# otiliastr/coper

Measured on AMD Instinct MI355X. Metric: scored triples/sec (1-vs-all), higher is better.
Workload: dtype fp16x3 (fp32 values split into two fp16 terms, 3 fp16 MFMAs per product, fp32 accumulate; comparisons closer than the split's error decided by the fp32 chain)

## Files before the change

### coper_amd/csrc/kernels_dense_fused_bf16.hip

```cpp
#include "bf16x3_chain.h"
#include "coper_internal.h"
#ifdef COPER_DBG_GROUP_CLK
#include <hip/hip_runtime.h>
__device__ unsigned long long g_group_clk[8];
extern "C" __attribute__((visibility("default"))) int coper_dbg_group_clock(unsigned long long* out) {
  return hipMemcpyFromSymbol(out, HIP_SYMBOL(g_group_clk), sizeof(unsigned long long) * 8) == hipSuccess ? 0 : 1;
}
#define GROUP_CLK(i) do { __syncthreads(); if (threadIdx.x == 0) g_group_clk[i] = wall_clock64(); } while (0)
#endif
#include "group_body.h"
#include "conv_fold.h"

namespace coper {

typedef float f32x4 __attribute__((ext_vector_type(4)));
typedef unsigned u32x4 __attribute__((ext_vector_type(4)));

#define MFMA16_BF16(a, b, c) S16_MFMA16(a, b, c)
#define MFMA16_X3(ahi, alo, bhi, blo, c) \
  { (c) = MFMA16_BF16(alo, bhi, c); (c) = MFMA16_BF16(ahi, blo, c); (c) = MFMA16_BF16(ahi, bhi, c); }


#ifndef COPER_FUSED_PMAX
#define COPER_FUSED_PMAX 3
#endif
#ifndef COPER_FUSED_PBUDGET
#define COPER_FUSED_PBUDGET 220
#endif


#define FW_DECL u32x4 W[P][NW][2]
#define FW_HI(s_, j_) W[s_][j_][0]
#define FW_LO(s_, j_) W[s_][j_][1]
#define FW_LO_RAW(s_, j_) W[s_][j_][1]
#define FW_PRE(s_)
#define FW_WREG3 (3 * NW * 8)

struct FusedConvArgs {
  const float* e1_rows;
  const int32_t* sorted_row;
  const int32_t* sorted_rid;
  const float* ent;
  const float* rel_emb;
  const float* conv_w;
  const float* conv_b;
  const float* scale;
  const float* shift;
  int per_rel_conv, d, r, in_w, in_hw, Wo, img_stride, x_exp;
  int img_exp;
  int64_t* chk;
  int w_div, w_rem;
  int32_t* bad;
};

#ifdef COPER_DBG_FUSED_CLOCK
__device__ unsigned long long g_fused_ph[8 * 2048];
extern "C" __attribute__((visibility("default"))) int coper_dbg_fused_phases(unsigned long long* out, int n) {
  return hipMemcpyFromSymbol(out, HIP_SYMBOL(g_fused_ph), sizeof(unsigned long long) * 8 * (n < 2048 ? n : 2048)) == hipSuccess ? 0 : 1;
}
#define FUSED_PH(i_)                                                                                            \
  do {                                                                                                          \
    const int w_ = blockIdx.x + gridDim.x * (blockIdx.y + gridDim.y * blockIdx.z);                              \
    if ((threadIdx.x & 63) == 0 && w_ < 2048) g_fused_ph[8 * w_ + (i_)] = __builtin_amdgcn_s_memrealtime();     \
  } while (0)
#else
#define FUSED_PH(i_) do { } while (0)
#endif
struct FusedFinConst {
  const int32_t* perm; const float* fc_b; const float* scale; const float* shift; const int32_t* w_exp; float* x3m;
  int per_rel_bias, x_exp, d, pad;
};
struct FusedFin {
  float* h_out; const FusedFinConst* c;
};
constexpr int FUSED_STAGE_WGS = 16;


__device__ __forceinline__ void fused_load_images(unsigned* __restrict__ img, const FusedConvArgs& A, int start, int n,
                                                  int t0, int t1) {
  const int wave = __builtin_amdgcn_readfirstlane(threadIdx.x >> 6), lane = threadIdx.x & 63;
  const int q0 = wave * 16;
  if (q0 < n) {
    int qi = q0 + (lane & 15);
    if (qi > n - 1) qi = n - 1;
    int my_row = A.sorted_row[start + qi], my_rid = A.sorted_rid[start + qi];
#ifdef COPER_DBG_NO_GROUP_CHK
    const bool chk = false;
#else
    const bool chk = A.chk != nullptr && (blockIdx.y | blockIdx.z) == 0;
#endif
    int64_t live_rel = 0, live_e1 = 0;
    const int chk_row = my_row, chk_rid = my_rid;
    if (chk) group_chk_issue(A.chk, start + qi, live_rel, live_e1);
#ifdef COPER_DBG_FUSED_NO_IMG
    my_row = -1;
#endif
    const float* base = A.e1_rows ? A.e1_rows : A.ent;
    const int len = t1 - t0, PD = (A.img_stride - 1) >> 1, eI = A.img_exp;
    auto fetch2 = [&](const int row, const int rid, const int t) -> float2 {
      if (t >= t1) return make_float2(0.f, 0.f);
      if (t < A.d) return row >= 0 ? *(const float2*)(base + (int64_t)row * A.d + t) : make_float2(0.f, 0.f);
      return *(const float2*)(A.rel_emb + (int64_t)rid * A.r + (t - A.d));
    };
    auto put2 = [&](const int q, const int pp, const float2 x) {
      unsigned short h0, l0, h1, l1;
      split1_s16(x3_scale(x.x, eI), h0, l0);
      split1_s16(x3_scale(x.y, eI), h1, l1);
      img[q * A.img_stride + pp] = (unsigned)h0 | ((unsigned)h1 << 16);
      img[q * A.img_stride + PD + pp] = (unsigned)l0 | ((unsigned)l1 << 16);
    };
    float2 v[16][2];
#pragma unroll
    for (int u = 0; u < 16; ++u) {
      const int row = __builtin_amdgcn_readlane(my_row, u), rid = __builtin_amdgcn_readlane(my_rid, u);
#pragma unroll
      for (int h = 0; h < 2; ++h) v[u][h] = fetch2(row, rid, t0 + 2 * (lane + 64 * h));
    }
#pragma unroll
    for (int u = 0; u < 16; ++u)
      if (q0 + u < n) {
#pragma unroll
        for (int h = 0; h < 2; ++h)
          if (2 * (lane + 64 * h) < len) put2(q0 + u, lane + 64 * h, v[u][h]);
        if (lane == 0) img[(q0 + u) * A.img_stride + 2 * PD] = 0u;
      }
    if (len > 256) {
      for (int u = 0; u < 16 && q0 + u < n; ++u) {
        const int row = __builtin_amdgcn_readlane(my_row, u), rid = __builtin_amdgcn_readlane(my_rid, u);
        for (int pp = 128 + lane; 2 * pp < len; pp += 64) put2(q0 + u, pp, fetch2(row, rid, t0 + 2 * pp));
      }
    }
    if (chk) group_chk_verdict(A.chk, live_rel, live_e1, chk_row, chk_rid);
  }
  asm volatile("s_waitcnt lgkmcnt(0)" ::: "memory");
  __builtin_amdgcn_s_barrier();
}

typedef unsigned fused_img_t;
template <int NFB, int NB, bool WNT>
__device__ __forceinline__ void fused_matrix_role(const uint4* __restrict__ xring, fused_img_t* __restrict__ img,
                                                  const uint4* __restrict__ Whi, const uint4* __restrict__ Wlo,
                                                  const FusedConvArgs& A, int64_t relw, int64_t relw_w, int start, int n, int fb0,
                                                  int nfb, int64_t ks32n, int64_t kb, int64_t ke, int t0, int t1,
                                                  float* __restrict__ zdst, int d_pad16, int wave, const FusedFin& Fn, int64_t ks32s) {
  constexpr int NFULL = NFB / 4;
  constexpr int REM = NFB % 4 ? 1 : 0;
  static_assert(NFB % 4 <= 1, "at most one left-over feature block");
  constexpr int NRQ = REM ? (NB + 3) / 4 : 0;
  constexpr int NW = NFULL + REM;
  constexpr int P = (COPER_FUSED_PMAX >= 3 && (NFULL * NB + NRQ) * 4 + FW_WREG3 + 44 <= COPER_FUSED_PBUDGET) ? 3 : 2;
  constexpr int XSTAGE = 2 * NB * 64;
  const int lane = threadIdx.x & 63;
  const int nk = (int)(ke - kb);
  const uint4* wp[NW][2];
#pragma unroll
  for (int j = 0; j < NW; ++j) {
    int fb = fb0 + (j < NFULL ? wave + 4 * j : 4 * NFULL);
    if (fb > nfb - 1) fb = nfb - 1;
    int64_t o = ((relw_w * nfb + fb) * ks32s + kb) * 64;
    wp[j][0] = Whi + o;
    wp[j][1] = (const uint4*)(Wlo + o);
  }
  FW_DECL;
#define FUSED_W_LOAD(p_) (WNT ? __builtin_nontemporal_load(p_) : *(p_))
#define W_ISSUE(s, kk)                                                                                 \
  {                                                                                                    \
    _Pragma("unroll") for (int j = 0; j < NW; ++j) {                                                   \
      FW_HI(s, j) = FUSED_W_LOAD((const u32x4*)(wp[j][0] + (int64_t)(kk)*64) + lane);                 \
      FW_LO_RAW(s, j) = FUSED_W_LOAD((const u32x4*)((const uint4*)wp[j][1] + (int64_t)(kk)*64) + lane); \
    }                                                                                                  \
  }
#pragma unroll
  for (int t = 0; t < P; ++t)
    if (t < nk) W_ISSUE(t, t);
  if (wave == 0) FUSED_PH(0);
  fused_load_images(img, A, start, n, t0, t1);
  if (wave == 0) FUSED_PH(1);
  f32x4 acc[NFULL][NB], accr[NRQ > 0 ? NRQ : 1];
#pragma unroll
  for (int j = 0; j < NFULL; ++j)
#pragma unroll
    for (int q = 0; q < NB; ++q) acc[j][q] = (f32x4){0.f, 0.f, 0.f, 0.f};
#pragma unroll
  for (int t = 0; t < NRQ; ++t) accr[t] = (f32x4){0.f, 0.f, 0.f, 0.f};
#ifdef COPER_DBG_FUSED_NO_MFMA
#define M_STEP(s2)                                                                                  \
  {                                                                                                 \
    __builtin_amdgcn_s_barrier();                                                                   \
    const uint4* xb = xring + ((s2)&1) * XSTAGE + lane;                                             \
    _Pragma("unroll") for (int j = 0; j < NW; ++j) {                                                \
      acc[0][0][0] += __uint_as_float(FW_HI((s2) % P, j)[0] ^ FW_LO_RAW((s2) % P, j)[1]);           \
      acc[0][0][1] += __uint_as_float(FW_HI((s2) % P, j)[2] ^ FW_LO_RAW((s2) % P, j)[0]);           \
    }                                                                                               \
    acc[0][0][2] += __uint_as_float(xb[0].x);                                                       \
  }
#else
#ifdef COPER_DBG_FUSED_NO_XREAD
#define M_LD(i_) make_uint4((unsigned)lane, (unsigned)(i_), 0x3c003c00u, 0x3c003c00u)
#else
#define M_LD(i_) xb[i_]
#endif
#ifndef COPER_FUSED_XPF
#define COPER_FUSED_XPF 2
#endif
#ifndef COPER_FUSED_XBUDGET
#define COPER_FUSED_XBUDGET 220
#endif
  constexpr int NV = NB + (NRQ > 0 ? 1 : 0);
  constexpr int XPF = (P == 3 && (NFULL * NB + NRQ) * 4 + FW_WREG3 + 44 > COPER_FUSED_XBUDGET) ? 1 : COPER_FUSED_XPF, XR = XPF + 1;
  const int qr = wave < NB ? wave : NB - 1;
#define M_LDV_H(v_) M_LD(((v_) < NB ? (v_) : qr) * 64)
#define M_LDV_L(v_) M_LD((NB + ((v_) < NB ? (v_) : qr)) * 64)
#define M_STEP(s2)                                                                                  \
  {                                                                                                 \
    FW_PRE((s2) % P)                                                                                \
    __builtin_amdgcn_s_barrier();                                                                   \
    const uint4* xb = xring + ((s2)&1) * XSTAGE + lane;                                             \
    uint4 bhq[XR], blq[XR];                                                                         \
    _Pragma("unroll") for (int v = 0; v < XPF && v < NV; ++v) { bhq[v] = M_LDV_H(v); blq[v] = M_LDV_L(v); } \
    __builtin_amdgcn_sched_group_barrier(0x100, 2 * (XPF < NV ? XPF : NV), 0);                      \
    _Pragma("unroll") for (int q = 0; q < NB; ++q) {                                                \
      if (q + XPF < NV) {                                                                           \
        bhq[(q + XPF) % XR] = M_LDV_H(q + XPF); blq[(q + XPF) % XR] = M_LDV_L(q + XPF);             \
        __builtin_amdgcn_sched_group_barrier(0x100, 2, 0);                                          \
      }                                                                                             \
      __builtin_amdgcn_sched_group_barrier(0x008, 3 * NFULL, 0);                                    \
      const uint4 bh = bhq[q % XR], bl = blq[q % XR];                                               \
      _Pragma("unroll") for (int j = 0; j < NFULL; ++j)                                             \
          acc[j][q] = MFMA16_BF16(FW_LO((s2) % P, j), bh, acc[j][q]);                               \
      _Pragma("unroll") for (int j = 0; j < NFULL; ++j)                                             \
          acc[j][q] = MFMA16_BF16(FW_HI((s2) % P, j), bl, acc[j][q]);                               \
      _Pragma("unroll") for (int j = 0; j < NFULL; ++j)                                             \
          acc[j][q] = MFMA16_BF16(FW_HI((s2) % P, j), bh, acc[j][q]);                               \
    }                                                                                               \
    _Pragma("unroll") for (int t = 0; t < NRQ; ++t) {                                               \
      const int q = wave + 4 * t < NB ? wave + 4 * t : NB - 1;  \
      uint4 bh, bl;                                                                                 \
      if (t == 0) { bh = bhq[NB % XR]; bl = blq[NB % XR]; }     \
      else { bh = M_LD(q * 64); bl = M_LD((NB + q) * 64); }                                         \
      accr[t] = MFMA16_BF16(FW_LO((s2) % P, NFULL), bh, accr[t]);                                   \
      accr[t] = MFMA16_BF16(FW_HI((s2) % P, NFULL), bl, accr[t]);                                   \
      accr[t] = MFMA16_BF16(FW_HI((s2) % P, NFULL), bh, accr[t]);                                   \
    }                                                                                               \
  }
#endif
  int k0 = 0;
  for (; k0 + 2 * P <= nk; k0 += 2 * P) {
#pragma unroll
    for (int s2 = 0; s2 < 2 * P; ++s2) {
      M_STEP(s2);
#ifndef COPER_DBG_FUSED_NO_W
      const int kn = k0 + s2 + P;
      W_ISSUE(s2 % P, kn < nk ? kn : 0);
#endif
    }
    if (k0 == 0 && wave == 0) FUSED_PH(2);
  }
#pragma unroll
  for (int s2 = 0; s2 < 2 * P - 1; ++s2) {
    if (k0 + s2 < nk) {
      M_STEP(s2);
#ifndef COPER_DBG_FUSED_NO_W
      if (k0 + s2 + P < nk) W_ISSUE(s2 % P, k0 + s2 + P);
#endif
    }
  }
#undef M_STEP
#undef W_ISSUE
  if (wave == 0) FUSED_PH(3);
#ifdef COPER_DBG_FUSED_NO_STORE
  if (acc[0][0][0] != 1.2345f) return;
#endif
  if (Fn.h_out) {
    const FusedFinConst Fc = *Fn.c;
    const int d = Fc.d;
    const int zexp = -((Fc.w_exp ? Fc.w_exp[Fc.per_rel_bias ? relw : 0] : 0) + Fc.x_exp);
    const float* bsrc = Fc.per_rel_bias ? Fc.fc_b + relw * d : Fc.fc_b;
    float m = 0.f;
    int qrow[NB];
#pragma unroll
    for (int q = 0; q < NB; ++q) {
      const int qi = q * 16 + (lane & 15);
      qrow[q] = qi < n ? Fc.perm[start + qi] : -1;
    }
    auto fin = [&](const f32x4& a, const int fb, const int q, const float4& b4, const float4& s4, const float4& t4) {
      const int k0 = fb * 16 + 4 * (lane >> 4);
      if (fb >= nfb || qrow[q] < 0 || k0 >= d) return;
      float z0 = 0.f, z1 = 0.f, z2 = 0.f, z3 = 0.f;
      z0 += a[0]; z1 += a[1]; z2 += a[2]; z3 += a[3];
      float4 v;
      v.x = fmaxf(fmaf(x3_scale(z0, zexp) + b4.x, s4.x, t4.x), 0.f);
      v.y = fmaxf(fmaf(x3_scale(z1, zexp) + b4.y, s4.y, t4.y), 0.f);
      v.z = fmaxf(fmaf(x3_scale(z2, zexp) + b4.z, s4.z, t4.z), 0.f);
      v.w = fmaxf(fmaf(x3_scale(z3, zexp) + b4.w, s4.w, t4.w), 0.f);
      m = fmaxf(m, fmaxf(fmaxf(v.x, v.y), fmaxf(v.z, v.w)));
      *(float4*)(Fn.h_out + (int64_t)qrow[q] * d + k0) = v;
    };
    auto quad = [&](const float* p, const int fb) -> float4 {
      const int k0 = fb * 16 + 4 * (lane >> 4);
      return (fb < nfb && k0 < d) ? *(const float4*)(p + k0) : make_float4(0.f, 0.f, 0.f, 0.f);
    };
#pragma unroll
    for (int j = 0; j < NFULL; ++j) {
      const int fb = fb0 + wave + 4 * j;
      const float4 b4 = quad(bsrc, fb), s4 = quad(Fc.scale, fb), t4 = quad(Fc.shift, fb);
#pragma unroll
      for (int q = 0; q < NB; ++q) fin(acc[j][q], fb, q, b4, s4, t4);
    }
    if (NRQ > 0) {
      const int fb = fb0 + 4 * NFULL;
      const float4 b4 = quad(bsrc, fb), s4 = quad(Fc.scale, fb), t4 = quad(Fc.shift, fb);
#pragma unroll
      for (int t = 0; t < NRQ; ++t) {
        const int q = wave + 4 * t;
        if (q < NB) {
          const int qi = q * 16 + (lane & 15);
          const int row = qi < n ? Fc.perm[start + qi] : -1;
          const int k0 = fb * 16 + 4 * (lane >> 4);
          if (fb < nfb && row >= 0 && k0 < d) {
            float z0 = 0.f, z1 = 0.f, z2 = 0.f, z3 = 0.f;
            z0 += accr[t][0]; z1 += accr[t][1]; z2 += accr[t][2]; z3 += accr[t][3];
            float4 v;
            v.x = fmaxf(fmaf(x3_scale(z0, zexp) + b4.x, s4.x, t4.x), 0.f);
            v.y = fmaxf(fmaf(x3_scale(z1, zexp) + b4.y, s4.y, t4.y), 0.f);
            v.z = fmaxf(fmaf(x3_scale(z2, zexp) + b4.z, s4.z, t4.z), 0.f);
            v.w = fmaxf(fmaf(x3_scale(z3, zexp) + b4.w, s4.w, t4.w), 0.f);
            m = fmaxf(m, fmaxf(fmaxf(v.x, v.y), fmaxf(v.z, v.w)));
            *(float4*)(Fn.h_out + (int64_t)row * d + k0) = v;
          }
        }
      }
    }
#pragma unroll
    for (int o = 32; o >= 1; o >>= 1) m = fmaxf(m, __shfl_xor(m, o));
    if (lane == 0 && m > 0.f)
      atomicMax((unsigned*)&Fc.x3m[(blockIdx.x + gridDim.x * blockIdx.z) & (X3M_SLOTS - 1)], __float_as_uint(m));
    return;
  }
#pragma unroll
  for (int j = 0; j < NFULL; ++j) {
    const int fb = fb0 + wave + 4 * j;
#pragma unroll
    for (int q = 0; q < NB; ++q) {
      const int qi = q * 16 + (lane & 15);
      if (fb < nfb && qi < n) {
        float* dst = zdst + (int64_t)(start + qi) * d_pad16 + fb * 16 + 4 * (lane >> 4);
        *(float4*)dst = make_float4(acc[j][q][0], acc[j][q][1], acc[j][q][2], acc[j][q][3]);
      }
    }
  }
#pragma unroll
  for (int t = 0; t < NRQ; ++t) {
    const int fb = fb0 + 4 * NFULL, q = wave + 4 * t;
    const int qi = q * 16 + (lane & 15);
    if (fb < nfb && q < NB && qi < n) {
      float* dst = zdst + (int64_t)(start + qi) * d_pad16 + fb * 16 + 4 * (lane >> 4);
      *(float4*)dst = make_float4(accr[t][0], accr[t][1], accr[t][2], accr[t][3]);
    }
  }
}

template <int NB>
__device__ __forceinline__ void fused_conv_role(uint4* __restrict__ xring, unsigned* __restrict__ img,
                                                const FusedConvArgs& A, int64_t relw, int start, int n, int64_t kb,
                                                int64_t ke, int i_lo, int t0, int t1, int cw) {
  constexpr int NFR = (NB + 3) / 4;
  constexpr int XSTAGE = 2 * NB * 64;
  const int lane = threadIdx.x & 63;
  const int nk = (int)(ke - kb);
  const int Wo = A.Wo, in_w = A.in_w, W2 = in_w >> 1;
  const int g = lane >> 4, m = lane & 15;
  const int PD = (A.img_stride - 1) >> 1;
  u32x4 aop[2];
  f32x4 cop[2];
  {
    const float* wsrc = A.per_rel_conv ? A.conv_w + relw * (int64_t)(9 * 32) : A.conv_w;
    const float* bsrc = A.per_rel_conv ? A.conv_b + relw * (int64_t)32 : A.conv_b;
    const int te = A.x_exp - A.img_exp;
#pragma unroll
    for (int u = 0; u < 2; ++u) {
      const int ch = 8 * (m >> 2) + 4 * u + (m & 3);
      const float sc = A.scale[ch];
      unsigned short th[9], tl[9];
#pragma unroll
      for (int k = 0; k < 9; ++k) split1_s16(x3_scale(wsrc[k * 32 + ch] * sc, te), th[k], tl[k]);
      unsigned short sl[8];
#pragma unroll
      for (int k = 0; k < 8; ++k) sl[k] = g == 2 ? tl[k] : th[k];
      if (g == 3) {
        sl[0] = th[8]; sl[1] = th[8]; sl[2] = tl[8];
#pragma unroll
        for (int k = 3; k < 8; ++k) sl[k] = 0;
      }
#pragma unroll
      for (int k = 0; k < 4; ++k) aop[u][k] = (unsigned)sl[2 * k] | ((unsigned)sl[2 * k + 1] << 16);
#pragma unroll
      for (int i = 0; i < 4; ++i) {
        const int c = 8 * g + 4 * u + i;
        cop[u][i] = x3_scale(fmaf(bsrc[c], A.scale[c], A.shift[c]), A.x_exp);
      }
    }
  }
  fused_load_images(img, A, start, n, t0, t1);
  if (cw == 0) FUSED_PH(5);
  int qown[NFR], qoth[NFR];
#pragma unroll
  for (int t = 0; t < NFR; ++t) {
    int qi = (cw + 4 * t) * 16 + m;
    if (qi > n - 1) qi = n - 1;
    qown[t] = qi * A.img_stride + (g == 1 ? PD : 0);
    qoth[t] = qi * A.img_stride + (g == 1 ? 0 : PD);
  }
  int poff = (int)(kb - (int64_t)i_lo * Wo);
  int cj = poff;
  for (int kk = 0; kk <= nk; ++kk) {
    if (kk > 0) {
      asm volatile("s_waitcnt lgkmcnt(0)" ::: "memory");
      __builtin_amdgcn_s_barrier();
    }
#ifdef COPER_DBG_FUSED_NO_CONV
    if (kk < 1) {
#else
    if (kk < nk) {
#endif
      const int pd = poff >> 1;
      const unsigned sh = (unsigned)(poff & 1) << 4;
#pragma unroll
      for (int t = 0; t < NFR; ++t) {
        if (cw + 4 * t < NB) {
          const unsigned* r = img + qown[t] + pd;
          const unsigned d00 = r[0], d01 = r[1], d10 = r[W2], d11 = r[W2 + 1], d20 = r[2 * W2], d21 = r[2 * W2 + 1];
          const unsigned o21 = img[qoth[t] + pd + 2 * W2 + 1];
          const unsigned a01 = __builtin_amdgcn_alignbit(d01, d00, sh), a2 = d01 >> sh;
          const unsigned b01 = __builtin_amdgcn_alignbit(d11, d10, sh), b2 = d11 >> sh;
          const unsigned c01 = __builtin_amdgcn_alignbit(d21, d20, sh), c2 = d21 >> sh;
          u32x4 bop;
          bop[0] = a01;
          bop[1] = __builtin_amdgcn_perm(b01, a2, 0x05040100u);
          bop[2] = __builtin_amdgcn_perm(b2, b01, 0x05040302u);
          bop[3] = c01;
          if (g == 3) {
            bop[0] = __builtin_amdgcn_perm(o21 >> sh, c2, 0x05040100u);
            bop[1] = c2 & 0xffffu;
          }
          const f32x4 y0 = MFMA16_BF16(aop[0], bop, cop[0]);
          const f32x4 y1 = MFMA16_BF16(aop[1], bop, cop[1]);
          float y[8];
#pragma unroll
          for (int i = 0; i < 4; ++i) {
            y[i] = __builtin_amdgcn_fmed3f(y0[i], 0.f, 65504.f);
            y[4 + i] = __builtin_amdgcn_fmed3f(y1[i], 0.f, 65504.f);
          }
          uint4 h4, l4;
          split8_pos_s16(y, h4, l4);
          uint4* dst = xring + (kk & 1) * XSTAGE + (cw + 4 * t) * 64 + lane;
          dst[0] = h4;
          dst[NB * 64] = l4;
        }
      }
      if (++cj == Wo) { cj = 0; poff += in_w - Wo + 1; } else { ++poff; }
    }
  }
}

#ifdef COPER_DBG_FUSED_CLOCK
__device__ unsigned long long g_fused_clk[3 * 2048];
extern "C" __attribute__((visibility("default"))) int coper_dbg_fused_clock(unsigned long long* out, int n) {
  return hipMemcpyFromSymbol(out, HIP_SYMBOL(g_fused_clk), sizeof(unsigned long long) * 3 * (n < 2048 ? n : 2048)) == hipSuccess ? 0 : 1;
}
#endif

template <int NFB, bool WNT>
__global__ __launch_bounds__(512) void k_dense_fused_bf16x3(const uint4* __restrict__ Whi, const uint4* __restrict__ Wlo,
                                                            FusedConvArgs A, const int32_t* __restrict__ tiles,
                                                            const int32_t* __restrict__ n_tiles, int64_t cap_small,
                                                            int nfb, int64_t ks32n, int nslices, int64_t Bcap,
                                                            int d_pad16, float* __restrict__ z_part, FusedFin Fn,
                                                            int n_special, const int32_t* __restrict__ stage_src, int64_t stage_n,
                                                            int64_t* __restrict__ stage_dst, int64_t ks32s, GroupJob J, int n_group,
                                                            const int32_t* __restrict__ post_src, int64_t post_n, int32_t* __restrict__ post_dst) {
  extern __shared__ uint4 fused_lds[];
  if ((int)blockIdx.x < n_special) {
    if (blockIdx.y | blockIdx.z) return;
    const int n_copy = n_special - n_group;
    if ((int)blockIdx.x >= n_copy) {
      GROUP_CLK(0);
      if (J.wait_for > 0) {
        if (threadIdx.x == 0) {
          for (int spin = 0; spin < (1 << 21) && __hip_atomic_load(J.ticket, __ATOMIC_RELAXED, __HIP_MEMORY_SCOPE_AGENT) < J.wait_for; ++spin)
            __builtin_amdgcn_s_sleep(16);
          (void)__hip_atomic_load(J.ticket, __ATOMIC_ACQUIRE, __HIP_MEMORY_SCOPE_AGENT);
          __hip_atomic_store(J.ticket, 0, __ATOMIC_RELAXED, __HIP_MEMORY_SCOPE_AGENT);
        }
        __syncthreads();
      }
      GROUP_CLK(1);
      group_role_body<512>(J, (int*)fused_lds);
      GROUP_CLK(5);
      return;
    }
    const int64_t nb = n_copy, b = (int64_t)blockIdx.x;
    if (post_n > 0) {
      const bool pvec = ((((uintptr_t)post_src) | ((uintptr_t)post_dst)) & 15) == 0;
      const int64_t p4 = pvec ? post_n / 4 : 0;
      for (int64_t i = b * 512 + threadIdx.x; i < p4; i += nb * 512) ((int4*)post_dst)[i] = ((const int4*)post_src)[i];
      for (int64_t i = 4 * p4 + b * 512 + threadIdx.x; i < post_n; i += nb * 512) post_dst[i] = post_src[i];
    }
    const bool vec = ((((uintptr_t)stage_src) | ((uintptr_t)stage_dst)) & 15) == 0;
    const int64_t n4 = vec ? stage_n / 4 : 0;
    auto copy4 = [&](int64_t lo, int64_t hi) {
      for (int64_t i = lo + b * 512 + threadIdx.x; i < hi; i += nb * 512) {
        const int4 v = ((const int4*)stage_src)[i];
        longlong2* o = (longlong2*)(stage_dst + 4 * i);
        o[0] = make_longlong2(v.x, v.y);
        o[1] = make_longlong2(v.z, v.w);
      }
    };
    const bool sig = n_group && J.wait_for > 0;
    int64_t f4 = sig ? (J.front + 3) / 4 : 0;
    if (f4 > n4 || f4 * 4 < J.front) f4 = 0;
    for (int64_t i = b * 512 + threadIdx.x; i < f4; i += nb * 512) {
      const int4 v = ((const int4*)stage_src)[i];
      int64_t* o = stage_dst + 4 * i;
      __hip_atomic_store(o + 0, (int64_t)v.x, __ATOMIC_RELAXED, __HIP_MEMORY_SCOPE_AGENT);
      __hip_atomic_store(o + 1, (int64_t)v.y, __ATOMIC_RELAXED, __HIP_MEMORY_SCOPE_AGENT);
      __hip_atomic_store(o + 2, (int64_t)v.z, __ATOMIC_RELAXED, __HIP_MEMORY_SCOPE_AGENT);
      __hip_atomic_store(o + 3, (int64_t)v.w, __ATOMIC_RELAXED, __HIP_MEMORY_SCOPE_AGENT);
    }
    if (sig && f4 == 0)
      for (int64_t i = b * 512 + threadIdx.x; i < J.front; i += nb * 512)
        __hip_atomic_store(stage_dst + i, (int64_t)stage_src[i], __ATOMIC_RELAXED, __HIP_MEMORY_SCOPE_AGENT);
    if (sig) {
      __syncthreads();
      if (threadIdx.x == 0) __hip_atomic_fetch_add(J.ticket, 1, __ATOMIC_RELEASE, __HIP_MEMORY_SCOPE_AGENT);
    }
    copy4(f4, n4);
    for (int64_t i = 4 * n4 + b * 512 + threadIdx.x; i < stage_n; i += nb * 512) stage_dst[i] = stage_src[i];
    return;
  }
  int tile = (int)blockIdx.x - n_special;
  const int32_t* tl;
  {
    const int nbig = n_tiles[1];
    if (tile < nbig) {
      tl = tiles + 4 * (cap_small + tile);
    } else {
      tile -= nbig;
      if (tile >= n_tiles[0]) return;
      tl = tiles + 4 * (int64_t)tile;
    }
  }
#ifdef COPER_DBG_FUSED_EXIT
  return;
#endif
  const int slice = blockIdx.y;
  const int fb0 = blockIdx.z * NFB;
  const int64_t relw = __builtin_amdgcn_readfirstlane(tl[0]);
  int64_t relw_w = relw;
  if (A.w_div > 1) {
    relw_w = (int)relw / A.w_div;
    if ((int)relw - (int)relw_w * A.w_div != A.w_rem && threadIdx.x == 0 && (blockIdx.y | blockIdx.z) == 0) atomicAdd(A.bad, (int)tl[2]);
  }
  const int start = __builtin_amdgcn_readfirstlane(tl[1]);
  const int n = __builtin_amdgcn_readfirstlane(tl[2]);
  const bool shared_w = __builtin_amdgcn_readfirstlane(tl[3]) != 0;
  const int64_t kb = ks32n * slice / nslices, ke = ks32n * (slice + 1) / nslices;
  float* zdst = z_part + (int64_t)slice * Bcap * d_pad16;
  const int nb = (n + 15) >> 4;
  const int wave = __builtin_amdgcn_readfirstlane(threadIdx.x >> 6);
#ifdef COPER_DBG_FUSED_CLOCK
  const unsigned long long dbg_t0 = __builtin_amdgcn_s_memrealtime();
#endif
  uint4* xring = fused_lds;
  unsigned* img = (unsigned*)(fused_lds + 2 * 16 * 64);
  const int i_lo = (int)(kb / A.Wo);
  const int t0 = i_lo * A.in_w;
  int t1 = ((int)((ke - 1) / A.Wo) + 3) * A.in_w;
  if (t1 > A.in_hw) t1 = A.in_hw;
#define TILE_WNT(x_) (x_)
#define BODY(NB_)                                                                                                      \
  if (wave < 4) {                                                                                                      \
    if (WNT && !shared_w)                                                                                              \
      fused_matrix_role<NFB, NB_, TILE_WNT(true)>(xring, img, Whi, Wlo, A, relw, relw_w, start, n, fb0, nfb, ks32n, kb, ke, t0, t1, zdst, \
                                                  d_pad16, wave, Fn, ks32s);                                           \
    else                                                                                                               \
      fused_matrix_role<NFB, NB_, TILE_WNT(false)>(xring, img, Whi, Wlo, A, relw, relw_w, start, n, fb0, nfb, ks32n, kb, ke, t0, t1, zdst, \
                                                   d_pad16, wave, Fn, ks32s);                                          \
  } else                                                                                                               \
    fused_conv_role<NB_>(xring, img, A, relw, start, n, kb, ke, i_lo, t0, t1, wave - 4);
  switch (nb) {
    case 1: BODY(1); break;
    case 2: BODY(2); break;
    case 3: BODY(3); break;
    case 4: BODY(4); break;
    case 5: BODY(5); break;
    case 6: BODY(6); break;
    case 7: BODY(7); break;
    default: BODY(8); break;
  }
#undef BODY
#ifdef COPER_DBG_FUSED_CLOCK
  if (threadIdx.x == 0) {
    const int w = blockIdx.x + gridDim.x * (blockIdx.y + gridDim.y * blockIdx.z);
    if (w < 2048) { g_fused_clk[3 * w] = (unsigned long long)n; g_fused_clk[3 * w + 1] = dbg_t0; g_fused_clk[3 * w + 2] = __builtin_amdgcn_s_memrealtime(); }
  }
#endif
}

static int fused_rows_max(const Dims& dm, int nslices) {
  int64_t ks32n = dm.F_pad / 32;
  int m = 0;
  for (int s = 0; s < nslices; ++s) {
    int64_t kb = ks32n * s / nslices, ke = ks32n * (s + 1) / nslices;
    if (ke <= kb) continue;
    int rows = (int)((ke - 1) / dm.Wo) - (int)(kb / dm.Wo) + 3;
    if (rows > m) m = rows;
  }
  return m;
}

bool dense_fused_supported(const coper_handle* h, int nslices) {
  const Dims& dm = h->dm;
  if (!(dm.fh == 3 && dm.fw == 3 && dm.C == 32) || dm.concat_rel) return false;
  if (dm.F != dm.F_pad || dm.F != (int64_t)dm.Ho * dm.Wo * 32) return false;
  if (dm.gen_conv && !dm.gen_fc) return false;
  if (!(dm.nfb == 13 || dm.nfb == 8 || dm.nfb == 16)) return false;
  if ((dm.in_w & 1) || (dm.d & 1) || (dm.stacked && (dm.r & 1))) return false;
  int stride = fused_rows_max(dm, nslices) * dm.in_w;
  stride |= 1;
  size_t lds = (size_t)2 * 16 * 64 * sizeof(uint4) + (size_t)128 * stride * sizeof(float);
  return lds <= 160 * 1024;
}

template <int NFB, bool WNT>
static void dense_fused_launch(coper_handle* h, PassCtx& ctx, const int64_t* e1, const int64_t* rel, const float* e1_rows, int64_t B,
                               int nslices, int zgroups, float* h_fin, hipStream_t s) {
  const Dims& dm = h->dm;
  const coper_handle::GroupSet& cur = h->grouping();
  FusedFin Fn;
  Fn.h_out = h_fin; Fn.c = (const FusedFinConst*)cur.fin.get();
  int64_t cap_small = (dm.gen_fc ? dm.R : 1) + 1;
  FusedConvArgs A;
  A.e1_rows = e1_rows; A.sorted_row = cur.sorted_row; A.sorted_rid = cur.sorted_rid;
  A.ent = h->lv.ent_emb->ptr;
  A.rel_emb = rel_emb_or_null(h);
  A.conv_w = conv_w(h);
  A.conv_b = conv_b(h);
  A.scale = h->conv_scale; A.shift = h->conv_shift; A.x_exp = h->x_exp; A.img_exp = h->img_exp;
  A.per_rel_conv = dm.gen_conv ? 1 : 0;
  A.d = dm.d; A.r = dm.r; A.in_w = dm.in_w; A.in_hw = dm.in_h * dm.in_w; A.Wo = dm.Wo;
  A.img_stride = (fused_rows_max(dm, nslices) * dm.in_w) | 1;
  A.chk = ctx.chk;
  A.w_div = h->w_div; A.w_rem = h->w_rem; A.bad = cur.rel_count + dm.R + 1;
  size_t lds = (size_t)2 * 16 * 64 * sizeof(uint4) + (size_t)128 * A.img_stride * sizeof(float);
  static uint64_t attr_done = 0;
  const uint64_t bit = 1ull << (h->cfg.device & 63);
  if (!(attr_done & bit)) {
    (void)hipFuncSetAttribute((const void*)k_dense_fused_bf16x3<NFB, WNT>, hipFuncAttributeMaxDynamicSharedMemorySize, 160 * 1024);
    attr_done |= bit;
  }
  const int n_tile_blocks = (int)(B / 128 + (cap_small - 1 < B ? cap_small - 1 : B) + 1);
  coper_handle::PassPipeline& pp = h->pipe;
  bool capturing = false;
  if (pp.stage.n > 0 || pp.post.n > 0 || ctx.gnext_ride) {
    hipStreamCaptureStatus cap = hipStreamCaptureStatusNone;
    if (hipStreamIsCapturing(s, &cap) != hipSuccess) { (void)hipGetLastError(); capturing = true; }
    else capturing = cap != hipStreamCaptureStatusNone;
  }
  const bool stage_now = pp.stage.n > 0 && !capturing;
  const bool post_now = pp.post.n > 0 && ctx.post_here && !capturing;
  GroupJob J = {};
  int n_group = 0;
  if (ctx.gnext_ride && !capturing) {
    const int64_t R = dm.gen_fc ? dm.R : 1;
    const int t = h->gcur == 1 ? 2 : 1;
    const coper_handle::GroupSet& g = h->gset[t];
    if (g.slab && pp.gnext.B <= h->ws_queries && group_role_lds_ints(R, 512) * sizeof(int) <= lds) {
      J.B = pp.gnext.B; J.R = R; J.R_all = dm.R; J.shard_lo = h->cfg.shard_lo; J.n_local = dm.n_local; J.cap_small = cap_small;
      J.count = g.rel_count; J.offset = g.rel_offset; J.tiles = g.tiles; J.n_tiles = g.n_tiles; J.perm = g.perm;
      J.sorted_row = g.sorted_row; J.sorted_rid = g.sorted_rid; J.inv_perm = g.inv_perm; J.x3m = g.x3m; J.x3m_slots = X3M_SLOTS;
      J.chk = g.chk;
      J.use_rel = dm.gen_fc ? 1 : 0; J.have_e1_rows = pp.gnext.rows;
      auto in_stage = [&](const int64_t* p) { return stage_now && p && p + J.B > pp.stage.dst && p < pp.stage.dst + pp.stage.n; };
      J.rel64 = pp.gnext.rel; J.e1_64 = pp.gnext.e1;
      J.ticket = h->group_done() + 1;
      J.wait_for = (in_stage(pp.gnext.rel) || in_stage(pp.gnext.e1)) ? FUSED_STAGE_WGS : 0;
      J.front = 0;
      if (in_stage(pp.gnext.rel)) J.front = (pp.gnext.rel + J.B) - pp.stage.dst;
      if (in_stage(pp.gnext.e1) && (pp.gnext.e1 + J.B) - pp.stage.dst > J.front) J.front = (pp.gnext.e1 + J.B) - pp.stage.dst;
      if (J.front > pp.stage.n) J.front = pp.stage.n;
      n_group = 1;
      pp.gdone.e1 = pp.gnext.e1; pp.gdone.rel = pp.gnext.rel; pp.gdone.B = pp.gnext.B; pp.gdone.rows = pp.gnext.rows;
      pp.gdone.done = true; pp.gdone.set = t;
    }
  }
  const int n_stage = (stage_now || post_now) ? FUSED_STAGE_WGS : 0;
  hipLaunchKernelGGL((k_dense_fused_bf16x3<NFB, WNT>), dim3((unsigned)(n_tile_blocks + n_group + n_stage), (unsigned)nslices, (unsigned)zgroups), dim3(512),
                     lds, s, (const uint4*)h->Wf16_hi, (const uint4*)h->Wf16_lo, A, cur.tiles, cur.n_tiles, cap_small, dm.nfb,
                     dm.F_pad / 32, nslices, h->ws_queries, dm.d_pad16, h->z_part, Fn, n_group + n_stage, pp.stage.src,
                     stage_now ? pp.stage.n : 0, pp.stage.dst, w16_ks_stride(dm), J, n_group, pp.post.src, post_now ? pp.post.n : 0, pp.post.dst);
  if (stage_now) pp.take_stage();
  if (post_now) pp.take_post();
}

int fused_fin_update(coper_handle* h, hipStream_t s) {
  const Dims& dm = h->dm;
  if (!h->enc_bf16 || !h->home.x3m || !h->home.perm) return COPER_OK;
  for (int i = 0; i < 3; ++i) {
    coper_handle::GroupSet& g = h->gset[i];
    if (i > 0 && !g.slab) continue;
    FusedFinConst c;
    c.perm = g.perm; c.fc_b = fc_b(h); c.scale = h->fc_scale; c.shift = h->fc_shift;
    c.w_exp = h->w_exp; c.x3m = g.x3m; c.per_rel_bias = dm.gen_fc ? 1 : 0; c.x_exp = h->x_exp; c.d = dm.d; c.pad = 0;
    int rc;
    if ((rc = g.fin.ensure(h, sizeof c, "fused finalize constants"))) return rc;
    COPER_HIP_TRY(h, hipMemcpyAsync(g.fin, &c, sizeof c, hipMemcpyHostToDevice, s));
    COPER_HIP_TRY(h, hipStreamSynchronize(s));
    g.fused_fin_perm = g.perm;
  }
  return COPER_OK;
}

bool dense_fused_finalizes(const coper_handle* h, int nslices, const float* h_out) {
  static const bool off = getenv("COPER_FUSED_NO_FINALIZE") != nullptr;
  const Dims& dm = h->dm;
  const float* fcb = fc_b(h);
  const coper_handle::GroupSet& g = h->grouping();
  return !off && h_out && nslices == 1 && g.x3m && g.fin && g.fused_fin_perm == g.perm && (dm.d & 3) == 0 &&
         ((((uintptr_t)h_out) | ((uintptr_t)fcb) | ((uintptr_t)h->fc_scale.get()) | ((uintptr_t)h->fc_shift.get())) & 15) == 0;
}

int launch_dense_fused_bf16(coper_handle* h, PassCtx& ctx, const int64_t* e1, const int64_t* rel, const float* e1_rows, int64_t B,
                            int nslices, float* h_fin, hipStream_t s) {
  if (!dense_fused_finalizes(h, nslices, h_fin)) h_fin = nullptr;
#ifndef COPER_FUSED_SPLIT_B
#define COPER_FUSED_SPLIT_B 2048
#endif
  const bool wnt = h->dm.gen_fc && B * 2 <= 128 * h->dm.R;
#define FUSED_GO(NFB_, Z_)                                                             \
  {                                                                                    \
    if (wnt) dense_fused_launch<NFB_, true>(h, ctx, e1, rel, e1_rows, B, nslices, Z_, h_fin, s);   \
    else dense_fused_launch<NFB_, false>(h, ctx, e1, rel, e1_rows, B, nslices, Z_, h_fin, s);      \
  }
  if (B <= COPER_FUSED_SPLIT_B / 2) FUSED_GO(4, (h->dm.nfb + 3) / 4)
  else if (h->dm.nfb == 13 && B > COPER_FUSED_SPLIT_B) FUSED_GO(13, 1)
  else FUSED_GO(8, (h->dm.nfb + 7) / 8)
#undef FUSED_GO
  COPER_HIP_TRY(h, hipGetLastError());
  return COPER_OK;
}

}
```

Before: 40.20 million.

## Prefetch finalize operands into LDS from conv waves during image load

The fused kernel's finalize epilogue used to read perm rows, bias, scale, shift, w_exp and the x3m pointer from global memory after the matrix loop. The conv-role waves now fetch these operands alongside the image loads and stage them in an extra 4 KB LDS block. The matrix-role epilogue then reads everything from LDS, taking dependent global loads off its tail. The cost is more LDS per block, which may reduce occupancy, plus extra register and instruction work on the conv waves. Finalize is also disabled when the enlarged LDS would exceed the limit.

```diff
diff --git a/coper_amd/csrc/kernels_dense_fused_bf16.hip b/coper_amd/csrc/kernels_dense_fused_bf16.hip
--- a/coper_amd/csrc/kernels_dense_fused_bf16.hip
+++ b/coper_amd/csrc/kernels_dense_fused_bf16.hip
@@ -73,17 +73,25 @@
 struct FusedFin {
   float* h_out; const FusedFinConst* c;
 };
+constexpr int FUSED_FIN_QUADS = 132;
+constexpr int FUSED_FIN_LDS = 4096;
+static_assert((FUSED_FIN_QUADS + 16 * 48) * 4 <= FUSED_FIN_LDS, "finalize operands fit their LDS block");
 constexpr int FUSED_STAGE_WGS = 16;
 
 
+struct FusedNoHook {
+  __device__ __forceinline__ void operator()() const {}
+};
+template <class Beside = FusedNoHook>
 __device__ __forceinline__ void fused_load_images(unsigned* __restrict__ img, const FusedConvArgs& A, int start, int n,
-                                                  int t0, int t1) {
+                                                  int t0, int t1, const Beside& beside = Beside()) {
   const int wave = __builtin_amdgcn_readfirstlane(threadIdx.x >> 6), lane = threadIdx.x & 63;
   const int q0 = wave * 16;
   if (q0 < n) {
     int qi = q0 + (lane & 15);
     if (qi > n - 1) qi = n - 1;
     int my_row = A.sorted_row[start + qi], my_rid = A.sorted_rid[start + qi];
+    beside();
 #ifdef COPER_DBG_NO_GROUP_CHK
     const bool chk = false;
 #else
@@ -131,6 +139,8 @@
       }
     }
     if (chk) group_chk_verdict(A.chk, live_rel, live_e1, chk_row, chk_rid);
+  } else {
+    beside();
   }
   asm volatile("s_waitcnt lgkmcnt(0)" ::: "memory");
   __builtin_amdgcn_s_barrier();
@@ -272,17 +282,12 @@
   if (acc[0][0][0] != 1.2345f) return;
 #endif
   if (Fn.h_out) {
-    const FusedFinConst Fc = *Fn.c;
-    const int d = Fc.d;
-    const int zexp = -((Fc.w_exp ? Fc.w_exp[Fc.per_rel_bias ? relw : 0] : 0) + Fc.x_exp);
-    const float* bsrc = Fc.per_rel_bias ? Fc.fc_b + relw * d : Fc.fc_b;
+    const unsigned* fl = img + 128 * A.img_stride;
+    const int zexp = (int)fl[128], d = (int)fl[129];
     float m = 0.f;
     int qrow[NB];
 #pragma unroll
-    for (int q = 0; q < NB; ++q) {
-      const int qi = q * 16 + (lane & 15);
-      qrow[q] = qi < n ? Fc.perm[start + qi] : -1;
-    }
+    for (int q = 0; q < NB; ++q) qrow[q] = (int)fl[q * 16 + (lane & 15)];
     auto fin = [&](const f32x4& a, const int fb, const int q, const float4& b4, const float4& s4, const float4& t4) {
       const int k0 = fb * 16 + 4 * (lane >> 4);
       if (fb >= nfb || qrow[q] < 0 || k0 >= d) return;
@@ -296,26 +301,24 @@
       m = fmaxf(m, fmaxf(fmaxf(v.x, v.y), fmaxf(v.z, v.w)));
       *(float4*)(Fn.h_out + (int64_t)qrow[q] * d + k0) = v;
     };
-    auto quad = [&](const float* p, const int fb) -> float4 {
-      const int k0 = fb * 16 + 4 * (lane >> 4);
-      return (fb < nfb && k0 < d) ? *(const float4*)(p + k0) : make_float4(0.f, 0.f, 0.f, 0.f);
+    auto quad = [&](const int a, const int fb) -> float4 {
+      return *(const float4*)(fl + FUSED_FIN_QUADS + ((fb - fb0) * 3 + a) * 16 + 4 * (lane >> 4));
     };
 #pragma unroll
     for (int j = 0; j < NFULL; ++j) {
       const int fb = fb0 + wave + 4 * j;
-      const float4 b4 = quad(bsrc, fb), s4 = quad(Fc.scale, fb), t4 = quad(Fc.shift, fb);
+      const float4 b4 = quad(0, fb), s4 = quad(1, fb), t4 = quad(2, fb);
 #pragma unroll
       for (int q = 0; q < NB; ++q) fin(acc[j][q], fb, q, b4, s4, t4);
     }
     if (NRQ > 0) {
       const int fb = fb0 + 4 * NFULL;
-      const float4 b4 = quad(bsrc, fb), s4 = quad(Fc.scale, fb), t4 = quad(Fc.shift, fb);
+      const float4 b4 = quad(0, fb), s4 = quad(1, fb), t4 = quad(2, fb);
 #pragma unroll
       for (int t = 0; t < NRQ; ++t) {
         const int q = wave + 4 * t;
         if (q < NB) {
-          const int qi = q * 16 + (lane & 15);
-          const int row = qi < n ? Fc.perm[start + qi] : -1;
+          const int row = (int)fl[q * 16 + (lane & 15)];
           const int k0 = fb * 16 + 4 * (lane >> 4);
           if (fb < nfb && row >= 0 && k0 < d) {
             float z0 = 0.f, z1 = 0.f, z2 = 0.f, z3 = 0.f;
@@ -333,8 +336,9 @@
     }
 #pragma unroll
     for (int o = 32; o >= 1; o >>= 1) m = fmaxf(m, __shfl_xor(m, o));
+    float* const x3m = (float*)((uintptr_t)fl[130] | ((uintptr_t)fl[131] << 32));
     if (lane == 0 && m > 0.f)
-      atomicMax((unsigned*)&Fc.x3m[(blockIdx.x + gridDim.x * blockIdx.z) & (X3M_SLOTS - 1)], __float_as_uint(m));
+      atomicMax((unsigned*)&x3m[(blockIdx.x + gridDim.x * blockIdx.z) & (X3M_SLOTS - 1)], __float_as_uint(m));
     return;
   }
 #pragma unroll
@@ -360,10 +364,48 @@
   }
 }
 
+struct FusedFinRegs {
+  unsigned row, we, q[3];
+};
+__device__ __forceinline__ void fused_fin_fetch(FusedFinRegs& r, const FusedFinConst& Fc, int64_t relw, int start, int n, int fb0, int nfb) {
+  const int tid = (int)threadIdx.x - 256;
+  const float* bsrc = Fc.per_rel_bias ? Fc.fc_b + relw * Fc.d : Fc.fc_b;
+  r.row = (unsigned)Fc.perm[start + (tid < n ? tid : n - 1)];
+  const int32_t* we = Fc.w_exp ? Fc.w_exp + (Fc.per_rel_bias ? relw : 0) : Fc.perm;
+  r.we = (unsigned)*we;
+#pragma unroll
+  for (int t = 0; t < 3; ++t) {
+    const int i = tid + 256 * t, a = (i % 48) >> 4;
+    int fb = fb0 + i / 48, k;
+    fb = fb < nfb ? fb : nfb - 1;
+    k = fb * 16 + (i & 15);
+    k = k < Fc.d ? k : Fc.d - 1;
+    const float* p = a == 0 ? bsrc : a == 1 ? Fc.scale : Fc.shift;
+    r.q[t] = __float_as_uint(p[k]);
+  }
+}
+__device__ __forceinline__ void fused_fin_put(unsigned* __restrict__ fin, const FusedFinRegs& r, const FusedFinConst& Fc, int n, int fb0,
+                                              int nfb, int nfbw) {
+  const int tid = (int)threadIdx.x - 256;
+  if (tid < FUSED_FIN_QUADS) {
+    const unsigned zexp = (unsigned)-((Fc.w_exp ? (int)r.we : 0) + Fc.x_exp);
+    fin[tid] = tid < 128 ? (tid < n ? r.row : ~0u)
+             : tid == 128 ? zexp
+             : tid == 129 ? (unsigned)Fc.d
+             : tid == 130 ? (unsigned)(uintptr_t)Fc.x3m : (unsigned)((uintptr_t)Fc.x3m >> 32);
+  }
+#pragma unroll
+  for (int t = 0; t < 3; ++t) {
+    const int i = tid + 256 * t, fb = fb0 + i / 48;
+    if (i < nfbw * 48) fin[FUSED_FIN_QUADS + i] = (fb < nfb && fb * 16 + (i & 15) < Fc.d) ? r.q[t] : 0u;
+  }
+}
+
 template <int NB>
 __device__ __forceinline__ void fused_conv_role(uint4* __restrict__ xring, unsigned* __restrict__ img,
                                                 const FusedConvArgs& A, int64_t relw, int start, int n, int64_t kb,
-                                                int64_t ke, int i_lo, int t0, int t1, int cw) {
+                                                int64_t ke, int i_lo, int t0, int t1, int cw, const FusedFin& Fn, int fb0, int nfb,
+                                                int nfbw) {
   constexpr int NFR = (NB + 3) / 4;
   constexpr int XSTAGE = 2 * NB * 64;
   const int lane = threadIdx.x & 63;
@@ -401,7 +443,14 @@
       }
     }
   }
-  fused_load_images(img, A, start, n, t0, t1);
+  if (Fn.h_out) {
+    FusedFinRegs finr;
+    const FusedFinConst Fc = *Fn.c;
+    fused_load_images(img, A, start, n, t0, t1, [&]() { fused_fin_fetch(finr, Fc, relw, start, n, fb0, nfb); });
+    fused_fin_put(img + 128 * A.img_stride, finr, Fc, n, fb0, nfb, nfbw);
+  } else {
+    fused_load_images(img, A, start, n, t0, t1);
+  }
   if (cw == 0) FUSED_PH(5);
   int qown[NFR], qoth[NFR];
 #pragma unroll
@@ -587,7 +636,7 @@
       fused_matrix_role<NFB, NB_, TILE_WNT(false)>(xring, img, Whi, Wlo, A, relw, relw_w, start, n, fb0, nfb, ks32n, kb, ke, t0, t1, zdst, \
                                                    d_pad16, wave, Fn, ks32s);                                          \
   } else                                                                                                               \
-    fused_conv_role<NB_>(xring, img, A, relw, start, n, kb, ke, i_lo, t0, t1, wave - 4);
+    fused_conv_role<NB_>(xring, img, A, relw, start, n, kb, ke, i_lo, t0, t1, wave - 4, Fn, fb0, nfb, NFB);
   switch (nb) {
     case 1: BODY(1); break;
     case 2: BODY(2); break;
@@ -619,6 +668,11 @@
   return m;
 }
 
+static size_t fused_lds_bytes(const Dims& dm, int nslices, bool fin) {
+  const int stride = (fused_rows_max(dm, nslices) * dm.in_w) | 1;
+  return (size_t)2 * 16 * 64 * sizeof(uint4) + (size_t)128 * stride * sizeof(float) + (fin ? FUSED_FIN_LDS : 0);
+}
+
 bool dense_fused_supported(const coper_handle* h, int nslices) {
   const Dims& dm = h->dm;
   if (!(dm.fh == 3 && dm.fw == 3 && dm.C == 32) || dm.concat_rel) return false;
@@ -626,10 +680,7 @@
   if (dm.gen_conv && !dm.gen_fc) return false;
   if (!(dm.nfb == 13 || dm.nfb == 8 || dm.nfb == 16)) return false;
   if ((dm.in_w & 1) || (dm.d & 1) || (dm.stacked && (dm.r & 1))) return false;
-  int stride = fused_rows_max(dm, nslices) * dm.in_w;
-  stride |= 1;
-  size_t lds = (size_t)2 * 16 * 64 * sizeof(uint4) + (size_t)128 * stride * sizeof(float);
-  return lds <= 160 * 1024;
+  return fused_lds_bytes(dm, nslices, false) <= 160 * 1024;
 }
 
 template <int NFB, bool WNT>
@@ -652,7 +703,7 @@
   A.img_stride = (fused_rows_max(dm, nslices) * dm.in_w) | 1;
   A.chk = ctx.chk;
   A.w_div = h->w_div; A.w_rem = h->w_rem; A.bad = cur.rel_count + dm.R + 1;
-  size_t lds = (size_t)2 * 16 * 64 * sizeof(uint4) + (size_t)128 * A.img_stride * sizeof(float);
+  const size_t lds = fused_lds_bytes(dm, nslices, h_fin != nullptr);
   static uint64_t attr_done = 0;
   const uint64_t bit = 1ull << (h->cfg.device & 63);
   if (!(attr_done & bit)) {
@@ -727,6 +778,7 @@
   const float* fcb = fc_b(h);
   const coper_handle::GroupSet& g = h->grouping();
   return !off && h_out && nslices == 1 && g.x3m && g.fin && g.fused_fin_perm == g.perm && (dm.d & 3) == 0 &&
+         fused_lds_bytes(dm, nslices, true) <= 160 * 1024 &&
          ((((uintptr_t)h_out) | ((uintptr_t)fcb) | ((uintptr_t)h->fc_scale.get()) | ((uintptr_t)h->fc_shift.get())) & 15) == 0;
 }
 
```

Result: no change. 40.52 million (median of 6 runs) (+0.8%).
